# MarineRoboticsGroup/mac

Hardware: AMD Instinct MI355X
Metric: frank_wolfe_iters_per_sec (higher is better)
Workload: dtype f64; 1 GPU; configs[3]: ER N=100000 ~2M candidates, chain fixed, K=10%; N=100000, m_candidates=2001737, K=200173, fixed_edges=99999, fw_iters=209, parallelism=single GPU

## Files before the change

mac_amd/csrc/kernels.h:

```cpp
#pragma once
#include "common.h"

namespace machip {

template <typename T>
struct CsrViewT {
    int n;
    const int* rowptr;
    const int* col;
    const T* val;
};
using CsrView = CsrViewT<double>;

struct PatternView {
    int n;
    const int* prow;
    const int* pcol;
    const int* pk;
    const double* pw;
};

struct LanState {
    int jA;
    int jB;
// ... 1025 lines not shown
                                                 const double* __restrict__ cw, const double* __restrict__ v,
                                                 long lo, long hi, double* __restrict__ g, PeerVecs all = PeerVecs(),
                                                 unsigned int* __restrict__ hist0 = nullptr) {
#pragma clang fp contract(off)
    __shared__ unsigned int lh[HIST ? kBins : 1];
    if (HIST) {
        for (int i = threadIdx.x; i < kBins; i += kBlock) lh[i] = 0;
        __syncthreads();
    }
    unsigned int cur = 0xffffffffu, run = 0;
    for (long k = lo + (long)blockIdx.x * kBlock + threadIdx.x; k < hi; k += (long)gridDim.x * kBlock) {
        const double d = v[ci[k]] - v[cj[k]];
        const double t = cw[k] * d;
        const double gk = t * d;
        if (all.n) { for (int q = 0; q < all.n; ++q) peer_store(all.v[q] + k, gk); }
        else g[k] = gk;
        if (HIST) {
            const unsigned int bin = (unsigned int)(f64_key(gk) >> sel_shift(0));
            if (bin == cur) ++run;
            else { if (run) atomicAdd(&lh[cur], run); cur = bin; run = 1; }
        }
    }
    if (HIST) {
        if (run) atomicAdd(&lh[cur], run);
        __syncthreads();
        unsigned int* hr = hist0 + (size_t)(blockIdx.x % kSelRep) * kBins;
        for (int i = threadIdx.x; i < kBins; i += kBlock)
            if (lh[i]) atomicAdd(&hr[i], lh[i]);
    }
    if (all.n) peer_drain();
}

template <int BLOCK, class LoadBin>
__device__ __forceinline__ void sel_close_pass(LoadBin load_bin, int pass, unsigned long long prefix, SelState* st,
                                               unsigned int* s_w ) {
    const int tid = threadIdx.x, wv = tid >> 6, ln = tid & 63;
    const int sh = sel_shift(pass), nb = sel_bits(pass);
    const long long kk = pass ? st->kk : st->k;
    const int nbins = 1 << nb;
    constexpr int per = kBins / BLOCK;
    unsigned int c[per];
    unsigned int tsum = 0;
#pragma unroll
    for (int q = 0; q < per; ++q) {
        const int bin = nbins - 1 - (tid * per + q);
        c[q] = bin >= 0 ? load_bin(bin) : 0u;
        tsum += c[q];
    }
    unsigned int x = tsum;
    for (int o = 1; o < 64; o <<= 1) { const unsigned int y = __shfl_up(x, o, kWave); if (ln >= o) x += y; }
    __syncthreads();
    if (ln == 63) s_w[wv] = x;
    __syncthreads();
    for (int q = 0; q < wv; ++q) x += s_w[q];
    const long long pre = (long long)x;
    if (pre >= kk && pre - (long long)tsum < kk) {
        long long rem = kk - (pre - (long long)tsum);
        int q = 0;
        for (; q < per; ++q) {
            if ((long long)c[q] >= rem) break;
            rem -= c[q];
        }
        const int bin = nbins - 1 - (tid * per + q);
        st->kk = rem;
        st->prefix = (prefix << nb) | (unsigned long long)bin;
        if (pass == 5) {
            st->T = (prefix << nb) | (unsigned long long)bin;
            st->cnt_eq = (long long)c[q];
        } else if ((long long)c[q] == rem) {
            st->T = ((prefix << nb) | (unsigned long long)bin) << sh;
            st->cnt_eq = rem;
            st->ticket[7] = 1u;
        }
    }
}

__global__ __launch_bounds__(1024) void k_sel_close0(unsigned int* __restrict__ hist, SelState* st) {
    __shared__ unsigned int s_w[1024 / 64];
    if (st->k <= 0) return;
    const unsigned int* rep = hist + 6 * kBins;
    sel_close_pass<1024>([rep](int bin) {
        unsigned int v[kSelRep];
#pragma unroll
        for (int r = 0; r < kSelRep; ++r) v[r] = rep[(size_t)r * kBins + bin];
        unsigned int a = 0;
#pragma unroll
        for (int r = 0; r < kSelRep; ++r) a += v[r];
        return a; }, 0, 0ull, st, s_w);
}

template <int U, int BLOCK>
__global__ __launch_bounds__(BLOCK) void k_sel_pass(const double* __restrict__ g, long m, int pass,
                                                    unsigned int* __restrict__ hist ,
                                                    SelState* st) {
    __shared__ unsigned int lh[kBins];
    __shared__ unsigned int s_last;
    __shared__ unsigned int s_w[BLOCK / 64];
    const int tid = threadIdx.x;
    if (pass && st->ticket[7]) return;
    for (int i = tid; i < kBins; i += BLOCK) lh[i] = 0;
    __syncthreads();
    const int sh = sel_shift(pass), nb = sel_bits(pass);
// ... 37 lines not shown
__global__ __launch_bounds__(1024) void k_sel_ties(const double* __restrict__ g, long m, SelState* st, int prefer_high) {
    __shared__ int s_cnt[16];
    __shared__ long long s_found;
    const long long need = st->kk;
    const long long eq = st->cnt_eq;
    if (st->k <= 0) { if (threadIdx.x == 0) st->tie_limit = prefer_high ? 0x7fffffffffffffffll : -1; return; }
    if (need >= eq) { if (threadIdx.x == 0) st->tie_limit = prefer_high ? -1 : 0x7fffffffffffffffll; return; }
    const unsigned long long T = st->T;
    const int tid = threadIdx.x, wv = tid >> 6, ln = tid & 63;
    if (tid == 0) s_found = -1;
    long long run = 0;
    for (long base = 0; base < m; base += 1024) {
        const long ii = base + tid;
        const long i = prefer_high ? m - 1 - ii : ii;
        const bool is = ii < m && f64_key(g[i]) == T;
        const unsigned long long bal = __ballot(is);
        __syncthreads();
        if (ln == 0) s_cnt[wv] = __popcll(bal);
        __syncthreads();
        int before = 0, tot = 0;
        for (int q = 0; q < 16; ++q) { if (q < wv) before += s_cnt[q]; tot += s_cnt[q]; }
        if (run + tot >= need) {
            const int rank = before + __popcll(bal & ((1ull << ln) - 1ull));
            if (is && run + rank + 1 == need) s_found = i;
            __syncthreads();
            if (tid == 0) st->tie_limit = s_found;
            return;
        }
        run += tot;
    }
    if (tid == 0) st->tie_limit = prefer_high ? -1 : 0x7fffffffffffffffll;
}

constexpr long kSelSmallMax = 32768;
__global__ __launch_bounds__(1024) void k_sel_small(const double* __restrict__ g, long m, long long k, SelState* st, int prefer_high) {
    __shared__ unsigned int lh[kBins];
    __shared__ unsigned int s_w[16];
    __shared__ unsigned long long s_prefix, s_T;
    __shared__ long long s_kk, s_eq, s_found;
    __shared__ int s_done, s_cnt[16];
    const int tid = threadIdx.x, wv = tid >> 6, ln = tid & 63;
    if (tid == 0) { s_prefix = 0; s_T = 0; s_kk = k; s_eq = 0; s_done = 0; s_found = -1; }
    __syncthreads();
    for (int pass = 0; pass < 6 && k > 0; ++pass) {
        if (s_done) break;
        for (int i = tid; i < kBins; i += 1024) lh[i] = 0;
        __syncthreads();
        const int sh = sel_shift(pass), nb = sel_bits(pass);
        const unsigned long long prefix = s_prefix;
        const unsigned int mask = (1u << nb) - 1u;
        unsigned int cur = 0xffffffffu, run = 0;
        for (long i = tid; i < m; i += 1024) {
            const unsigned long long key = f64_key(g[i]);
            if (pass == 0 || (key >> (sh + nb)) == prefix) {
                const unsigned int bin = (unsigned int)(key >> sh) & mask;
                if (bin == cur) ++run;
                else { if (run) atomicAdd(&lh[cur], run); cur = bin; run = 1; }
            }
        }
        if (run) atomicAdd(&lh[cur], run);
        __syncthreads();
        const long long kk = s_kk;
        const int nbins = 1 << nb;
        unsigned int c[2], tsum = 0;
        for (int q = 0; q < 2; ++q) { const int bin = nbins - 1 - (tid * 2 + q); c[q] = bin >= 0 ? lh[bin] : 0u; tsum += c[q]; }
        unsigned int x = tsum;
        for (int o = 1; o < 64; o <<= 1) { const unsigned int y = __shfl_up(x, o, kWave); if (ln >= o) x += y; }
        if (ln == 63) s_w[wv] = x;
        __syncthreads();
        for (int q = 0; q < wv; ++q) x += s_w[q];
        const long long pre = (long long)x;
        if (pre >= kk && pre - (long long)tsum < kk) {
            long long rem = kk - (pre - (long long)tsum);
            int q = 0;
            for (; q < 2; ++q) { if ((long long)c[q] >= rem) break; rem -= c[q]; }
            const int bin = nbins - 1 - (tid * 2 + q);
            s_kk = rem;
            s_prefix = (prefix << nb) | (unsigned long long)bin;
            if (pass == 5) { s_T = (prefix << nb) | (unsigned long long)bin; s_eq = (long long)c[q]; }
            else if ((long long)c[q] == rem) { s_T = ((prefix << nb) | (unsigned long long)bin) << sh; s_eq = rem; s_done = 1; }
        }
        __syncthreads();
    }
    const long long need = s_kk, eq = s_eq;
    const unsigned long long T = s_T;
    if (tid == 0) {
        st->prefix = s_prefix; st->kk = need; st->cnt_eq = eq; st->T = T; st->k = k;
        for (int i = 0; i < 7; ++i) st->ticket[i] = 0;
        st->ticket[7] = (unsigned int)s_done;
    }
    if (k <= 0) { if (tid == 0) st->tie_limit = prefer_high ? 0x7fffffffffffffffll : -1; return; }
    if (need >= eq) { if (tid == 0) st->tie_limit = prefer_high ? -1 : 0x7fffffffffffffffll; return; }
    long long runs = 0;
    for (long base = 0; base < m; base += 1024) {
        const long ii = base + tid;
        const long i = prefer_high ? m - 1 - ii : ii;
        const bool is = ii < m && f64_key(g[i]) == T;
        const unsigned long long bal = __ballot(is);
        __syncthreads();
        if (ln == 0) s_cnt[wv] = __popcll(bal);
        __syncthreads();
        int before = 0, tot = 0;
        for (int q = 0; q < 16; ++q) { if (q < wv) before += s_cnt[q]; tot += s_cnt[q]; }
        if (runs + tot >= need) {
            const int rank = before + __popcll(bal & ((1ull << ln) - 1ull));
            if (is && runs + rank + 1 == need) s_found = i;
            __syncthreads();
            if (tid == 0) st->tie_limit = s_found;
            return;
        }
        runs += tot;
    }
    if (tid == 0) st->tie_limit = prefer_high ? -1 : 0x7fffffffffffffffll;
}

__global__ __launch_bounds__(kBlock) void k_fw_final(const double* __restrict__ g, const double* __restrict__ x,
                                                     long m, const SelState* __restrict__ st, double gamma,
                                                     double* __restrict__ x_next, double* __restrict__ s_out,
                                                     double* __restrict__ part ,
                                                     double tol = 0.0, unsigned long long* __restrict__ xbits_next = nullptr) {
#pragma clang fp contract(off)
    __shared__ double sm[4];
    const unsigned long long T = st->T;
    const long long lim = st->tie_limit;
    const bool none = st->k <= 0;
    double d = 0.0, q = 0.0;
    for (long i = (long)blockIdx.x * kBlock + threadIdx.x; i < m; i += (long)gridDim.x * kBlock) {
        const double gi = g[i];
        const unsigned long long key = f64_key(gi);
        const double s = (!none && (key > T || (key == T && (long long)i <= lim))) ? 1.0 : 0.0;
        if (s_out) s_out[i] = s;
        if (x) {
            const double xi = x[i];
            const double diff = s - xi;
            d += gi * diff;
            q += gi * gi;
            if (x_next) {
                const double step = gamma * diff;
                const double xn = xi + step;
                x_next[i] = xn;
                if (xbits_next) {
                    const unsigned long long bal = __ballot(xn > tol);
                    if ((threadIdx.x & 63) == 0) xbits_next[i >> 6] = bal;
                }
            }
        }
// ... 74 lines not shown
```

mac_amd/csrc/machip.hip:

```cpp
#include <rccl/rccl.h>
#include <unistd.h>

#include <algorithm>
#include <atomic>
#include <cmath>
#include <chrono>
#include <condition_variable>
#include <functional>
#include <future>
#include <memory>
#include <mutex>
#include <numeric>
#include <thread>
#include <vector>

#include "solver.h"
#include "esp.h"
#include "esp_free.h"
#include "esp_tree.h"
#include "esp_select.h"
#include "esp_relax.h"
#include "esp_exchange.h"
#include "esp_exchange_edge.h"
#include "eig_exchange.h"
// ... 51 lines not shown
    }
    void abort() {
        std::lock_guard<std::mutex> lk(mu);
        broken = true;
        cv.notify_all();
    }
};

struct machip_problem {
    int device = 0;
    hipStream_t stream = nullptr;
    int n = 0;
    long m = 0, m_pad = 0;
    double tol_sel = 1e-10;
    int *prow = nullptr, *pcol = nullptr, *pk = nullptr;
    double* pw = nullptr;
    long P = 0;
    int asm_G = 16, asm_rpb = 1, asm_grid = 1;
    int *ci = nullptr, *cj = nullptr;
    double* cw = nullptr;
    double *x = nullptr, *x_next = nullptr, *g = nullptr, *s = nullptr, *scratch_m = nullptr;
    int *cnt = nullptr, *blk_sum = nullptr, *rowptr = nullptr, *col = nullptr;
    double *val = nullptr, *blk_lnorm = nullptr;
    unsigned long long *xb = nullptr, *xb_next = nullptr;
    bool xb_valid = false, xb_next_valid = false;
    long nnz = 0, support = 0;
    int maxlen = 0;
    double lnorm = 0.0;
    bool assembled = false, have_vec = false, csr_only = false;
    bool band_dups_ok = true;
    unsigned int* hist = nullptr;
    SelState* sel = nullptr;
    double* part_fw = nullptr;
    int* h_int = nullptr;
    double* h_dbl = nullptr;
    int* d_hint = nullptr;
    double* d_hdbl = nullptr;
    Solver sol;
    ncclComm_t comm = nullptr;
    std::shared_ptr<LocalGroup> lgroup;
    bool first_collective_pending = false;
    hipEvent_t ev_g0 = nullptr, ev_g1 = nullptr, ev_g2 = nullptr;
    bool ev_g_valid = false;
    std::unique_ptr<IpcGroup> ipcg;
    int rank = 0, nranks = 1;
    bool is_lane = false, lane_fw_ready = false;
    std::vector<machip_problem*> lanes;
    unsigned long start_version = 0;
    unsigned long seen_start_version = ~0ul;

    CsrView csr() const { return CsrView{n, rowptr, col, val}; }
    PatternView pattern() const { return PatternView{n, prow, pcol, pk, pw}; }
};

static int create_lane_stream(const Options& opt, int device, hipStream_t* out) {
    if (OPT(lane_queues, 0) == 0) {
        hipDeviceProp_t prop;
        if (hipGetDeviceProperties(&prop, device) == hipSuccess && prop.multiProcessorCount > 0) {
            const int words = (prop.multiProcessorCount + 31) / 32;
            std::vector<uint32_t> mask((size_t)words, 0xffffffffu);
            if (prop.multiProcessorCount % 32) mask.back() = (1u << (prop.multiProcessorCount % 32)) - 1u;
            if (hipExtStreamCreateWithCUMask(out, (uint32_t)words, mask.data()) == hipSuccess) return MACHIP_OK;
            (void)hipGetLastError();
        }
    }
    HIP_TRY(hipStreamCreateWithFlags(out, hipStreamNonBlocking));
// ... 115 lines not shown
        p->xb_valid = true;
    }
    switch (p->asm_G) {
        case 4: launch_asm<4>(p, S); break;
        case 8: launch_asm<8>(p, S); break;
        case 16: launch_asm<16>(p, S); break;
        case 32: launch_asm<32>(p, S); break;
        default: launch_asm<64>(p, S); break;
    }
    HIP_TRY(hipGetLastError());
    const int gb = p->asm_grid;
    HIP_TRY(hipStreamSynchronize(p->stream));
    long nnz = 0, supp = 0;
    int maxlen = 0;
    double ln = 0.0;
    for (int b = 0; b < gb; ++b) {
        nnz += p->h_int[b]; supp += p->h_int[kAsmGrid + b]; maxlen = std::max(maxlen, p->h_int[2 * kAsmGrid + b]);
        ln = std::max(ln, p->h_dbl[b]);
    }
    p->nnz = nnz; p->support = supp / 2; p->lnorm = ln; p->maxlen = maxlen;
    p->assembled = true;
    return MACHIP_OK;
}

int alloc_common(machip_problem* p, int vbudget_mb = 0) {
    ST_TRY(p->sol.init(p->n, p->stream, vbudget_mb));
    HIP_TRY(hipHostMalloc((void**)&p->h_int, sizeof(int) * 3 * kAsmGrid, hipHostMallocMapped));
    HIP_TRY(hipHostMalloc((void**)&p->h_dbl, sizeof(double) * std::max(4 * kMaxGrid, kAsmGrid), hipHostMallocMapped));
    HIP_TRY(hipHostGetDevicePointer((void**)&p->d_hint, p->h_int, 0));
    HIP_TRY(hipHostGetDevicePointer((void**)&p->d_hdbl, p->h_dbl, 0));
    return MACHIP_OK;
}

int select_on(machip_problem* p, const double* keys, long k, SelState* st, int prefer_high, bool hist0_done = false) {
    const Options& opt = p->sol.opt;
    const long m = p->m;
    if (k < 0) k = 0;
    if (k > m) k = m;
    if (m <= kSelSmallMax && OPT(sel_small, 1)) {
        k_sel_small<<<1, 1024, 0, p->stream>>>(keys, m, (long long)k, st, prefer_high);
        HIP_TRY(hipGetLastError());
        return MACHIP_OK;
    }
    if (!hist0_done) k_sel_init<<<1, 1024, 0, p->stream>>>(st, (long long)k, p->hist, 6 * kBins);
    if (k > 0) {
        constexpr int B = 1024, U = 4;
        const int grid = (int)std::max<long>(1, std::min<long>(128, (m + (long)B * U - 1) / ((long)B * U)));
        if (hist0_done) k_sel_close0<<<1, 1024, 0, p->stream>>>(p->hist, st);
        for (int pass = hist0_done ? 1 : 0; pass < 6; ++pass) k_sel_pass<U, B><<<grid, B, 0, p->stream>>>(keys, m, pass, p->hist, st);
    }
    k_sel_ties<<<1, 1024, 0, p->stream>>>(keys, m, st, prefer_high);
    HIP_TRY(hipGetLastError());
    return MACHIP_OK;
}

int select_topk(machip_problem* p, long k, bool hist0_done = false) { return select_on(p, p->g, k, p->sel, 0, hist0_done); }

void shard_plan(long m, int nranks, int rank, long* lo, long* hi, long* shard) {
    const long sh = nranks > 0 ? (m + nranks - 1) / nranks : m;
    *shard = sh;
    *lo = std::min(m, sh * rank);
    *hi = std::min(m, *lo + sh);
}

int local_allgather(machip_problem* p, long shard) {
    LocalGroup& G = *p->lgroup;
    HIP_TRY(hipStreamSynchronize(p->stream));
    if (!G.barrier()) return fail(MACHIP_RCCL_ERROR, "in-process communicator was shut down by another rank");
    for (int r = 0; r < G.nranks; ++r)
        if (r != p->rank)
            HIP_TRY(hipMemcpyAsync(p->g + shard * r, G.g[(size_t)r] + shard * r, sizeof(double) * (size_t)shard,
                                   hipMemcpyDeviceToDevice, p->stream));
    HIP_TRY(hipStreamSynchronize(p->stream));
    if (!G.barrier()) return fail(MACHIP_RCCL_ERROR, "in-process communicator was shut down by another rank");
    return MACHIP_OK;
}

int compute_gradient(machip_problem* p, bool have_vec_now = false, long fuse_k = -1, bool* fused = nullptr) {
    const Options& opt = p->sol.opt;
    if (!p->have_vec && !have_vec_now) return fail(MACHIP_BAD_ARG, "no Fiedler vector on the device: call machip_fiedler first");
    const long m = p->m;
    long lo = 0, hi = m, shard = m;
    if (p->nranks > 1) shard_plan(m, p->nranks, p->rank, &lo, &hi, &shard);
    const bool ipc_gather = p->nranks > 1 && !p->comm && p->ipcg;
    if (ipc_gather) {
        k_ipc_pubwait<<<1, 64, 0, p->stream>>>(p->ipcg->view, 3);
    }
    const bool timed = p->nranks > 1;
    if (timed) {
        if (!p->ev_g0) { HIP_TRY(hipEventCreate(&p->ev_g0)); HIP_TRY(hipEventCreate(&p->ev_g1)); HIP_TRY(hipEventCreate(&p->ev_g2)); }
        p->ev_g_valid = false;
        HIP_TRY(hipEventRecord(p->ev_g0, p->stream));
    }
    if (hi > lo) {
        const int grid = (int)std::min<long>(kMaxGrid * 4, (hi - lo + kBlock - 1) / kBlock);
        PeerVecs all;
        if (ipc_gather) { all.n = p->ipcg->nranks; for (int q = 0; q < all.n; ++q) all.v[q] = p->ipcg->g[q]; }
        const bool fuse = fuse_k > 0 && p->nranks <= 1 && m > kSelSmallMax && OPT(sel_fuse, 1) != 0;
        if (fused) *fused = fuse;
        if (fuse) {
            k_sel_init<<<1, 1024, 0, p->stream>>>(p->sel, (long long)std::min(fuse_k, m), p->hist, (6 + kSelRep) * kBins);
            k_grad<true><<<grid, kBlock, 0, p->stream>>>(p->ci, p->cj, p->cw, p->sol.yvec, lo, hi, p->g, all, p->hist + 6 * kBins);
        } else k_grad<false><<<grid, kBlock, 0, p->stream>>>(p->ci, p->cj, p->cw, p->sol.yvec, lo, hi, p->g, all);
        HIP_TRY(hipGetLastError());
    }
    if (timed) HIP_TRY(hipEventRecord(p->ev_g1, p->stream));
    if (ipc_gather) {
        k_ipc_pubwait<<<1, 64, 0, p->stream>>>(p->ipcg->view, 2);
        HIP_TRY(hipGetLastError());
        HIP_TRY(hipEventRecord(p->ev_g2, p->stream));
        p->ev_g_valid = true;
        return MACHIP_OK;
    }
    if (p->nranks > 1) {
        if (p->comm) {
            NCCL_TRY(ncclAllGather(p->g + shard * p->rank, p->g, (size_t)shard, ncclDouble, p->comm, p->stream));
            if (p->first_collective_pending) {
                p->first_collective_pending = false;
                const auto t0 = std::chrono::steady_clock::now();
                const double lim = rccl_timeout_s();
                for (;;) {
                    const hipError_t q = hipStreamQuery(p->stream);
                    if (q == hipSuccess) break;
                    if (q != hipErrorNotReady) return fail(MACHIP_HIP_ERROR, std::string("first ncclAllGather: ") + hipGetErrorString(q));
                    ncclResult_t ar = ncclSuccess;
                    if (ncclCommGetAsyncError(p->comm, &ar) == ncclSuccess && ar != ncclSuccess && ar != ncclInProgress)
                        return fail(MACHIP_RCCL_ERROR, std::string("first ncclAllGather failed asynchronously: ") + ncclGetErrorString(ar));
                    if (std::chrono::duration<double>(std::chrono::steady_clock::now() - t0).count() > lim) {
                        (void)ncclCommAbort(p->comm);
                        p->comm = nullptr;
                        return fail(MACHIP_RCCL_ERROR, "first ncclAllGather of rank " + std::to_string(p->rank) + " of " + std::to_string(p->nranks) +
                                    " did not complete within " + std::to_string((int)lim) + " s: communicator aborted");
                    }
                    std::this_thread::sleep_for(std::chrono::microseconds(200));
// ... 131 lines not shown
                const int a = std::min(fi[e], fj[e]), b = std::max(fi[e], fj[e]);
                if (a >= 0 && b < n && b == a + 1 && fw[e] > 0.0) has[(size_t)a] = 1;
            }
            long cnt = 0;
            for (int64_t i = 0; i + 1 < n; ++i) cnt += has[(size_t)i];
            p->sol.chain_like = cnt >= (long)(0.98 * (double)(n - 1));
            p->sol.chain_edges = cnt;
        }
        return MACHIP_OK;
    };
    st = body();
    if (st != MACHIP_OK) { machip_destroy(p); return st; }
    *out = p;
    return MACHIP_OK;
}

void machip_destroy(machip_problem* p) {
    if (!p) return;
    for (machip_problem* q : p->lanes) machip_destroy(q);
    p->lanes.clear();
    (void)hipSetDevice(p->device);
    if (p->stream) (void)hipStreamSynchronize(p->stream);
    if (p->is_lane) { p->prow = p->pcol = p->pk = nullptr; p->pw = nullptr; p->ci = p->cj = nullptr; p->cw = nullptr; }
    if (p->comm) (void)ncclCommDestroy(p->comm);
    if (p->lgroup) p->lgroup->abort();
    if (p->ipcg) {
        IpcGroup& G = *p->ipcg;
        if (!G.clean_exit) { k_ipc_abort<<<1, 64, 0, p->stream>>>(G.view); (void)hipStreamSynchronize(p->stream); }
        p->sol.ipc = nullptr;
        p->ipcg.reset();
    }
    p->sol.destroy();
    void* ptrs[] = {p->prow, p->pcol, p->pk, p->pw, p->ci, p->cj, p->cw, p->x, p->x_next, p->g, p->s, p->scratch_m, p->cnt,
                    p->blk_sum, p->rowptr, p->col, p->val, p->blk_lnorm, p->xb, p->xb_next, p->hist, p->sel, p->part_fw};
    for (void* q : ptrs) if (q) (void)hipFree(q);
    for (hipEvent_t e : {p->ev_g0, p->ev_g1, p->ev_g2}) if (e) (void)hipEventDestroy(e);
    if (p->h_int) (void)hipHostFree(p->h_int);
    if (p->h_dbl) (void)hipHostFree(p->h_dbl);
    if (p->stream) (void)hipStreamDestroy(p->stream);
    delete p;
}

int machip_set_x(machip_problem* p, const double* x) {
    if (!p || !x || p->csr_only) return fail(MACHIP_BAD_ARG, "machip_set_x: bad handle or NULL x");
    HIP_TRY(hipSetDevice(p->device));
    HIP_TRY(hipMemcpyAsync(p->x, x, sizeof(double) * (size_t)p->m, hipMemcpyHostToDevice, p->stream));
    HIP_TRY(hipStreamSynchronize(p->stream));
    p->assembled = false; p->xb_valid = false;
    return MACHIP_OK;
}

int machip_get_x(machip_problem* p, double* x) {
    if (!p || !x || p->csr_only) return fail(MACHIP_BAD_ARG, "machip_get_x: bad handle or NULL x");
    HIP_TRY(hipSetDevice(p->device));
    HIP_TRY(hipMemcpyAsync(x, p->x, sizeof(double) * (size_t)p->m, hipMemcpyDeviceToHost, p->stream));
    HIP_TRY(hipStreamSynchronize(p->stream));
    return MACHIP_OK;
}

int machip_assemble(machip_problem* p, int64_t* nnz_out) {
    if (!p) return fail(MACHIP_BAD_ARG, "NULL handle");
    HIP_TRY(hipSetDevice(p->device));
    ST_TRY(assemble(p));
    if (nnz_out) *nnz_out = p->nnz;
    return MACHIP_OK;
}

// ... 686 lines not shown
                st = machip_fw_commit(q);
            }
            if (st == MACHIP_OK) st = machip_get_x(q, X_out + (size_t)b * m);
            if (st == MACHIP_OK && R_out) st = machip_round_nearest(q, ks[b], round_decimals, R_out + (size_t)b * m);
            upper[b] = u; iters[b] = done; status[b] = st;
            if (st != MACHIP_OK && st != MACHIP_NOT_CONVERGED && st != MACHIP_DISCONNECTED) {
                lane_status[(size_t)l] = st; lane_err[(size_t)l] = g_err;
                return;
            }
        }
    };
    std::vector<std::thread> th;
    for (int l = 1; l < nl; ++l) th.emplace_back(work, l);
    work(0);
    for (auto& t : th) t.join();
    for (int l = 0; l < nl; ++l)
        if (lane_status[(size_t)l] != MACHIP_OK) return fail((machip_status)lane_status[(size_t)l], lane_err[(size_t)l]);
    return MACHIP_OK;
}

int machip_set_option(machip_problem* p, const char* name, int64_t value) {
    const int id = option_id(name);
    if (id < 0) return fail(MACHIP_BAD_ARG, std::string("machip_set_option: unknown option '") + (name ? name : "(null)") + "'");
    const long v = value == INT64_MIN ? kOptAuto : (long)value;
    if (!p) { default_options().v[id] = v; return MACHIP_OK; }
    p->sol.opt.v[id] = v;
    for (machip_problem* q : p->lanes) q->sol.opt.v[id] = v;
    return MACHIP_OK;
}

int machip_get_option(machip_problem* p, const char* name, int64_t* value) {
    const int id = option_id(name);
    if (id < 0 || !value) return fail(MACHIP_BAD_ARG, "machip_get_option: unknown option or NULL output");
    const long v = p ? p->sol.opt.v[id] : default_options().v[id];
    *value = v == kOptAuto ? INT64_MIN : (int64_t)v;
    return MACHIP_OK;
}

const char* machip_option_name(int i) { return (i >= 0 && i < kNumOpts) ? option_names()[i] : nullptr; }

int machip_comm_timing(machip_problem* p, double* grad_us, double* exchange_us) {
    if (!p || !grad_us || !exchange_us) return fail(MACHIP_BAD_ARG, "machip_comm_timing: NULL argument");
    *grad_us = 0.0; *exchange_us = 0.0;
    if (!p->ev_g_valid) return fail(MACHIP_BAD_ARG, "machip_comm_timing: no sharded gradient has been computed on this handle");
    HIP_TRY(hipSetDevice(p->device));
    HIP_TRY(hipEventSynchronize(p->ev_g2));
    float a = 0.f, b = 0.f;
    HIP_TRY(hipEventElapsedTime(&a, p->ev_g0, p->ev_g1));
    HIP_TRY(hipEventElapsedTime(&b, p->ev_g1, p->ev_g2));
    *grad_us = 1e3 * (double)a; *exchange_us = 1e3 * (double)b;
    return MACHIP_OK;
}

int machip_solve_mode(machip_problem* p, int64_t* closures) {
    if (!p) return -1;
    if (closures) *closures = p->sol.last_wb_s;
    return p->sol.last_mode;
}

int machip_comm_drop(machip_problem* p) {
    if (!p) return fail(MACHIP_BAD_ARG, "machip_comm_drop: NULL handle");
    if (p->lgroup) return fail(MACHIP_BAD_ARG, "machip_comm_drop: in-process communicators end with their handles");
    HIP_TRY(hipSetDevice(p->device));
    (void)hipStreamSynchronize(p->stream);
    if (p->ipcg) { p->sol.ipc = nullptr; p->ipcg.reset(); }
    if (p->comm) { (void)ncclCommAbort(p->comm); p->comm = nullptr; }
// ... 343 lines not shown
```

mac_amd/csrc/options.h:

```cpp
#pragma once
#include <climits>
#include <cstdlib>
#include <cstring>
#include <mutex>
#include <string>

namespace machip {

#define MACHIP_OPTION_LIST(X)                                                                                                      \
                                                                                                          \
    X(solver) X(graph) X(debug) X(chunk) X(chunk_near) X(sched) X(near_x10) X(trigger_pct) X(classic_n) X(persist) X(pchunk)      \
    X(spec_epilogue) X(spec_slack_pct) X(f32_switch_e9) X(tailless) X(stream) X(stream_trigger_pct) X(stream_retry_pct) X(stream_look) X(stream_margin) X(stream_window) X(stream_far) X(start_land) X(start_pow) X(start_floor_e6) X(start_land_pr_permille) X(start_land_min_mean10)                                                                \
                                                                        \
    X(spmv) X(g) X(unroll) X(block) X(maxgrid) X(defer) X(tpr) X(ell)                                                              \
                                                                                                            \
    X(panel) X(panel_min_n) X(panel_min_mean10) X(panel_multi_min_mean10) X(panel_np) X(panel_nb) X(panel_b2) X(panel_g2)         \
    X(panel_cells) X(panel_maxcells) X(panel_band) X(panel_u) X(panel_u_amp) X(pan32) X(pan32_switch_e9) X(panel_ops) X(panel_rev)                                                                               \
                                                                                                 \
    X(woodbury) X(wb_max) X(wb_hard) X(wb_lane_max) X(exact_big) X(exact_switch) X(gj_look_min) X(lob_density_pct) X(lob_chunk)   \
    X(lob_patience) X(lob_small_s) X(lob_fuse)                                                                                     \
     \
    X(sel_small) X(sel_fuse) X(asm_g) X(asm_maxgrid) X(vbudget_mb) X(vcap) X(lanes) X(lane_vbudget_mb) X(lane_queues) X(shard_eig) X(ipc_panel) \
    X(rccl_timeout_s)                                                                                                              \
               \
    X(esp_free_split)                                                                                                              \
       \
    X(esp_xch_lds_kb) X(esp_xch_max_mb) X(esp_xch_profile)                                                                         \
                                                       \
    X(eig_xch_max_mb)                                                                                                              \
                                                                                                            \
    X(eig_free_rows) X(eig_free_split)

enum OptId {
#define X(n) kOpt_##n,
    MACHIP_OPTION_LIST(X)
#undef X
    kNumOpts
};

constexpr long kOptAuto = LONG_MIN;

inline const char* const* option_names() {
    static const char* const names[] = {
#define X(n) #n,
        MACHIP_OPTION_LIST(X)
#undef X
        nullptr};
    return names;
}
inline int option_id(const char* name) {
    if (!name) return -1;
    const char* const* nm = option_names();
    for (int i = 0; i < kNumOpts; ++i) if (!strcmp(nm[i], name)) return i;
    return -1;
}

// ... 43 lines not shown
```

Before: 135.1 iter/s.

## Replace multi-pass radix top-k select with two-kernel coarse bucket plus candidate list

Adds a two-kernel top-k selection path for the fused gradient histogram case. The first kernel closes pass 0 from the replicated histogram and builds a coarse 8-bit sub-histogram. The second compacts the candidates in the chosen bucket into a small global list, finishes the radix walk and tie resolution in one block, and zeroes histograms so the next iteration can skip k_sel_init. This is meant to replace several full-array radix passes and extra launches per Frank-Wolfe iteration. If the bucket holds more than the list capacity it falls back to a single-block whole-array walk, which could be slow.

Result: no change. 134.5 iter/s (-0.4%).

```diff
diff --git a/mac_amd/csrc/kernels.h b/mac_amd/csrc/kernels.h
--- a/mac_amd/csrc/kernels.h
+++ b/mac_amd/csrc/kernels.h
@@ -1081,11 +1081,9 @@
 }
 
 template <int BLOCK, class LoadBin>
-__device__ __forceinline__ void sel_close_pass(LoadBin load_bin, int pass, unsigned long long prefix, SelState* st,
-                                               unsigned int* s_w ) {
+__device__ __forceinline__ bool sel_close_find(LoadBin load_bin, int nb, long long kk, unsigned int* s_w ,
+                                               int* bin_out, long long* rem_out, unsigned int* cnt_out) {
     const int tid = threadIdx.x, wv = tid >> 6, ln = tid & 63;
-    const int sh = sel_shift(pass), nb = sel_bits(pass);
-    const long long kk = pass ? st->kk : st->k;
     const int nbins = 1 << nb;
     constexpr int per = kBins / BLOCK;
     unsigned int c[per];
@@ -1103,20 +1101,33 @@
     __syncthreads();
     for (int q = 0; q < wv; ++q) x += s_w[q];
     const long long pre = (long long)x;
-    if (pre >= kk && pre - (long long)tsum < kk) {
-        long long rem = kk - (pre - (long long)tsum);
-        int q = 0;
-        for (; q < per; ++q) {
-            if ((long long)c[q] >= rem) break;
-            rem -= c[q];
-        }
-        const int bin = nbins - 1 - (tid * per + q);
+    if (!(pre >= kk && pre - (long long)tsum < kk)) return false;
+    long long rem = kk - (pre - (long long)tsum);
+    int q = 0;
+    for (; q < per; ++q) {
+        if ((long long)c[q] >= rem) break;
+        rem -= c[q];
+    }
+    *bin_out = nbins - 1 - (tid * per + q);
+    *rem_out = rem;
+    *cnt_out = c[q];
+    return true;
+}
+
+template <int BLOCK, class LoadBin>
+__device__ __forceinline__ void sel_close_pass(LoadBin load_bin, int pass, unsigned long long prefix, SelState* st,
+                                               unsigned int* s_w ) {
+    const int sh = sel_shift(pass), nb = sel_bits(pass);
+    int bin = 0;
+    long long rem = 0;
+    unsigned int cnt = 0;
+    if (sel_close_find<BLOCK>(load_bin, nb, pass ? st->kk : st->k, s_w, &bin, &rem, &cnt)) {
         st->kk = rem;
         st->prefix = (prefix << nb) | (unsigned long long)bin;
         if (pass == 5) {
             st->T = (prefix << nb) | (unsigned long long)bin;
-            st->cnt_eq = (long long)c[q];
-        } else if ((long long)c[q] == rem) {
+            st->cnt_eq = (long long)cnt;
+        } else if ((long long)cnt == rem) {
             st->T = ((prefix << nb) | (unsigned long long)bin) << sh;
             st->cnt_eq = rem;
             st->ticket[7] = 1u;
@@ -1220,65 +1231,53 @@
     if (tid == 0) st->tie_limit = prefer_high ? -1 : 0x7fffffffffffffffll;
 }
 
-constexpr long kSelSmallMax = 32768;
-__global__ __launch_bounds__(1024) void k_sel_small(const double* __restrict__ g, long m, long long k, SelState* st, int prefer_high) {
-    __shared__ unsigned int lh[kBins];
-    __shared__ unsigned int s_w[16];
-    __shared__ unsigned long long s_prefix, s_T;
-    __shared__ long long s_kk, s_eq, s_found;
-    __shared__ int s_done, s_cnt[16];
-    const int tid = threadIdx.x, wv = tid >> 6, ln = tid & 63;
-    if (tid == 0) { s_prefix = 0; s_T = 0; s_kk = k; s_eq = 0; s_done = 0; s_found = -1; }
-    __syncthreads();
-    for (int pass = 0; pass < 6 && k > 0; ++pass) {
-        if (s_done) break;
-        for (int i = tid; i < kBins; i += 1024) lh[i] = 0;
+struct SelWalk {
+    unsigned long long prefix, T;
+    long long kk, eq, found;
+    int done;
+    unsigned int lh[kBins], s_w[16];
+    int s_cnt[16];
+};
+
+template <class KeyAt>
+__device__ __forceinline__ void sel_walk(KeyAt key_at, long cnt, int pass0, SelWalk* w) {
+    const int tid = threadIdx.x;
+    for (int pass = pass0; pass < 6; ++pass) {
+        if (w->done) break;
+        for (int i = tid; i < kBins; i += 1024) w->lh[i] = 0;
         __syncthreads();
         const int sh = sel_shift(pass), nb = sel_bits(pass);
-        const unsigned long long prefix = s_prefix;
+        const unsigned long long prefix = w->prefix;
+        const long long kk = w->kk;
         const unsigned int mask = (1u << nb) - 1u;
         unsigned int cur = 0xffffffffu, run = 0;
-        for (long i = tid; i < m; i += 1024) {
-            const unsigned long long key = f64_key(g[i]);
+        for (long i = tid; i < cnt; i += 1024) {
+            const unsigned long long key = key_at(i);
             if (pass == 0 || (key >> (sh + nb)) == prefix) {
                 const unsigned int bin = (unsigned int)(key >> sh) & mask;
                 if (bin == cur) ++run;
-                else { if (run) atomicAdd(&lh[cur], run); cur = bin; run = 1; }
+                else { if (run) atomicAdd(&w->lh[cur], run); cur = bin; run = 1; }
             }
         }
-        if (run) atomicAdd(&lh[cur], run);
+        if (run) atomicAdd(&w->lh[cur], run);
         __syncthreads();
-        const long long kk = s_kk;
-        const int nbins = 1 << nb;
-        unsigned int c[2], tsum = 0;
-        for (int q = 0; q < 2; ++q) { const int bin = nbins - 1 - (tid * 2 + q); c[q] = bin >= 0 ? lh[bin] : 0u; tsum += c[q]; }
-        unsigned int x = tsum;
-        for (int o = 1; o < 64; o <<= 1) { const unsigned int y = __shfl_up(x, o, kWave); if (ln >= o) x += y; }
-        if (ln == 63) s_w[wv] = x;
+        const unsigned int* lh = w->lh;
+        int bin = 0;
+        long long rem = 0;
+        unsigned int c = 0;
+        if (sel_close_find<1024>([lh](int b) { return lh[b]; }, nb, kk, w->s_w, &bin, &rem, &c)) {
+            w->kk = rem;
+            w->prefix = (prefix << nb) | (unsigned long long)bin;
+            if (pass == 5) { w->T = (prefix << nb) | (unsigned long long)bin; w->eq = (long long)c; }
+            else if ((long long)c == rem) { w->T = ((prefix << nb) | (unsigned long long)bin) << sh; w->eq = rem; w->done = 1; }
+        }
         __syncthreads();
-        for (int q = 0; q < wv; ++q) x += s_w[q];
-        const long long pre = (long long)x;
-        if (pre >= kk && pre - (long long)tsum < kk) {
-            long long rem = kk - (pre - (long long)tsum);
-            int q = 0;
-            for (; q < 2; ++q) { if ((long long)c[q] >= rem) break; rem -= c[q]; }
-            const int bin = nbins - 1 - (tid * 2 + q);
-            s_kk = rem;
-            s_prefix = (prefix << nb) | (unsigned long long)bin;
-            if (pass == 5) { s_T = (prefix << nb) | (unsigned long long)bin; s_eq = (long long)c[q]; }
-            else if ((long long)c[q] == rem) { s_T = ((prefix << nb) | (unsigned long long)bin) << sh; s_eq = rem; s_done = 1; }
-        }
-        __syncthreads();
-    }
-    const long long need = s_kk, eq = s_eq;
-    const unsigned long long T = s_T;
-    if (tid == 0) {
-        st->prefix = s_prefix; st->kk = need; st->cnt_eq = eq; st->T = T; st->k = k;
-        for (int i = 0; i < 7; ++i) st->ticket[i] = 0;
-        st->ticket[7] = (unsigned int)s_done;
-    }
-    if (k <= 0) { if (tid == 0) st->tie_limit = prefer_high ? 0x7fffffffffffffffll : -1; return; }
-    if (need >= eq) { if (tid == 0) st->tie_limit = prefer_high ? -1 : 0x7fffffffffffffffll; return; }
+    }
+}
+
+__device__ __forceinline__ void sel_ties_scan(const double* __restrict__ g, long m, unsigned long long T, long long need,
+                                              int prefer_high, SelWalk* w, SelState* st) {
+    const int tid = threadIdx.x, wv = tid >> 6, ln = tid & 63;
     long long runs = 0;
     for (long base = 0; base < m; base += 1024) {
         const long ii = base + tid;
@@ -1286,20 +1285,224 @@
         const bool is = ii < m && f64_key(g[i]) == T;
         const unsigned long long bal = __ballot(is);
         __syncthreads();
-        if (ln == 0) s_cnt[wv] = __popcll(bal);
+        if (ln == 0) w->s_cnt[wv] = __popcll(bal);
         __syncthreads();
         int before = 0, tot = 0;
-        for (int q = 0; q < 16; ++q) { if (q < wv) before += s_cnt[q]; tot += s_cnt[q]; }
+        for (int q = 0; q < 16; ++q) { if (q < wv) before += w->s_cnt[q]; tot += w->s_cnt[q]; }
         if (runs + tot >= need) {
             const int rank = before + __popcll(bal & ((1ull << ln) - 1ull));
-            if (is && runs + rank + 1 == need) s_found = i;
+            if (is && runs + rank + 1 == need) w->found = i;
             __syncthreads();
-            if (tid == 0) st->tie_limit = s_found;
+            if (tid == 0) st->tie_limit = w->found;
             return;
         }
         runs += tot;
     }
     if (tid == 0) st->tie_limit = prefer_high ? -1 : 0x7fffffffffffffffll;
+}
+
+__device__ __forceinline__ void sel_whole(const double* __restrict__ g, long m, long long k, int pass0, int prefer_high,
+                                          SelWalk* w, SelState* st) {
+    const int tid = threadIdx.x;
+    if (k > 0) sel_walk([g](long i) { return f64_key(g[i]); }, m, pass0, w);
+    const long long need = w->kk, eq = w->eq;
+    const unsigned long long T = w->T;
+    if (tid == 0) {
+        st->prefix = w->prefix; st->kk = need; st->cnt_eq = eq; st->T = T; st->k = k;
+        for (int i = 0; i < 7; ++i) st->ticket[i] = 0;
+        st->ticket[7] = (unsigned int)w->done;
+    }
+    if (k <= 0) { if (tid == 0) st->tie_limit = prefer_high ? 0x7fffffffffffffffll : -1; return; }
+    if (need >= eq) { if (tid == 0) st->tie_limit = prefer_high ? -1 : 0x7fffffffffffffffll; return; }
+    sel_ties_scan(g, m, T, need, prefer_high, w, st);
+}
+
+constexpr long kSelSmallMax = 32768;
+__global__ __launch_bounds__(1024) void k_sel_small(const double* __restrict__ g, long m, long long k, SelState* st, int prefer_high) {
+    __shared__ SelWalk w;
+    if (threadIdx.x == 0) { w.prefix = 0; w.T = 0; w.kk = k; w.eq = 0; w.done = 0; w.found = -1; }
+    __syncthreads();
+    sel_whole(g, m, k, 0, prefer_high, &w, st);
+}
+
+constexpr int kSelList = 8192;
+constexpr int kSelCoarse = 8;
+struct SelTwo {
+    unsigned int cursor;
+    unsigned int ticket_a, ticket_b;
+    unsigned int whole;
+    unsigned int whole_runs;
+    unsigned int bucket;
+    unsigned int cprefix;
+    long long ckk;
+};
+
+template <int U, int BLOCK>
+__global__ __launch_bounds__(BLOCK) void k_sel_two_a(const double* __restrict__ g, long m, long long k,
+                                                      unsigned int* __restrict__ hist , SelState* st, SelTwo* tw) {
+    constexpr int kCoarse = 1 << kSelCoarse;
+    __shared__ unsigned int lh[kCoarse];
+    __shared__ unsigned int s_w[BLOCK / 64];
+    __shared__ unsigned int s_last, s_cnt[2];
+    __shared__ int s_bin[2];
+    __shared__ long long s_rem[2];
+    const int tid = threadIdx.x;
+    const unsigned int* rep = hist + 6 * kBins;
+    unsigned int* gh = hist + kBins;
+    {
+        int bin = 0;
+        long long rem = 0;
+        unsigned int cnt = 0;
+        if (sel_close_find<BLOCK>([rep](int b) {
+                unsigned int v[kSelRep];
+#pragma unroll
+                for (int r = 0; r < kSelRep; ++r) v[r] = rep[(size_t)r * kBins + b];
+                unsigned int a = 0;
+#pragma unroll
+                for (int r = 0; r < kSelRep; ++r) a += v[r];
+                return a; }, sel_bits(0), k, s_w, &bin, &rem, &cnt)) { s_bin[0] = bin; s_rem[0] = rem; s_cnt[0] = cnt; }
+    }
+    for (int i = tid; i < kCoarse; i += BLOCK) lh[i] = 0;
+    __syncthreads();
+    const unsigned long long bin0 = (unsigned long long)s_bin[0];
+    const long long rem0 = s_rem[0];
+    const bool done0 = (long long)s_cnt[0] == rem0;
+    if (!done0) {
+        constexpr int sh = 53 - kSelCoarse;
+        unsigned int cur = 0xffffffffu, run = 0;
+        for (long i0 = (long)blockIdx.x * (BLOCK * U) + tid; i0 < m; i0 += (long)gridDim.x * (BLOCK * U)) {
+            double gv[U];
+#pragma unroll
+            for (int q = 0; q < U; ++q) { const long i = i0 + (long)q * BLOCK; gv[q] = g[i < m ? i : m - 1]; }
+#pragma unroll
+            for (int q = 0; q < U; ++q) {
+                if (i0 + (long)q * BLOCK >= m) continue;
+                const unsigned long long key = f64_key(gv[q]);
+                if ((key >> 53) == bin0) {
+                    const unsigned int bin = (unsigned int)(key >> sh) & (kCoarse - 1);
+                    if (bin == cur) ++run;
+                    else { if (run) atomicAdd(&lh[cur], run); cur = bin; run = 1; }
+                }
+            }
+        }
+        if (run) atomicAdd(&lh[cur], run);
+        __syncthreads();
+        unsigned int seen = 0;
+        for (int i = tid; i < kCoarse; i += BLOCK)
+            if (lh[i]) seen |= __hip_atomic_fetch_add(&gh[i], lh[i], __ATOMIC_RELAXED, __HIP_MEMORY_SCOPE_AGENT);
+        asm volatile("" ::"v"(seen));
+    }
+    __syncthreads();
+    if (tid == 0)
+        s_last = (__hip_atomic_fetch_add(&tw->ticket_a, 1u, __ATOMIC_ACQ_REL, __HIP_MEMORY_SCOPE_AGENT) == gridDim.x - 1);
+    __syncthreads();
+    if (!s_last) return;
+    if (!done0) {
+        int bin = 0;
+        long long rem = 0;
+        unsigned int cnt = 0;
+        if (sel_close_find<BLOCK>([gh](int b) { return __hip_atomic_load(&gh[b], __ATOMIC_RELAXED, __HIP_MEMORY_SCOPE_AGENT); },
+                                  kSelCoarse, rem0, s_w, &bin, &rem, &cnt)) { s_bin[1] = bin; s_rem[1] = rem; s_cnt[1] = cnt; }
+    }
+    __syncthreads();
+    for (int i = tid; i < kCoarse; i += BLOCK) gh[i] = 0u;
+    if (tid == 0) {
+        st->prefix = bin0; st->kk = rem0; st->k = k;
+        st->cnt_eq = done0 ? rem0 : 0; st->T = done0 ? bin0 << 53 : 0ull;
+        st->tie_limit = done0 ? 0x7fffffffffffffffll : -1;
+        for (int i = 0; i < 7; ++i) st->ticket[i] = 0;
+        st->ticket[7] = done0 ? 1u : 0u;
+        const unsigned int bucket = done0 ? 0u : s_cnt[1];
+        const unsigned int whole = bucket > (unsigned int)kSelList ? 1u : 0u;
+        tw->whole = whole;
+        tw->whole_runs += whole;
+        tw->bucket = bucket;
+        tw->cprefix = done0 ? 0u : (unsigned int)((bin0 << kSelCoarse) | (unsigned long long)s_bin[1]);
+        tw->ckk = done0 ? 0 : s_rem[1];
+        tw->ticket_a = 0u;
+    }
+}
+
+template <int U, int BLOCK>
+__global__ __launch_bounds__(BLOCK) void k_sel_two_b(const double* __restrict__ g, long m, unsigned int* __restrict__ hist, SelState* st,
+                                                      SelTwo* tw, unsigned long long* lkey , unsigned int* lidx ) {
+    static_assert(BLOCK == 1024, "sel_walk is written for 1 024 threads");
+    __shared__ SelWalk w;
+    __shared__ unsigned int s_idx[kSelList];
+    __shared__ unsigned int s_last, s_n, s_base;
+    const int tid = threadIdx.x, ln = tid & 63;
+    for (int i = blockIdx.x * BLOCK + tid; i < kSelRep * kBins; i += gridDim.x * BLOCK) hist[6 * kBins + i] = 0u;
+    if (st->ticket[7]) return;
+    if (tid == 0) { w.prefix = st->prefix; w.T = 0; w.kk = st->kk; w.eq = 0; w.done = 0; w.found = -1; s_n = 0; }
+    if (tw->whole) {
+        if (blockIdx.x) return;
+        __syncthreads();
+        sel_whole(g, m, st->k, 1, 0, &w, st);
+        return;
+    }
+    __syncthreads();
+    const unsigned long long cprefix = tw->cprefix;
+    for (long i0 = (long)blockIdx.x * (BLOCK * U) + tid; i0 < m; i0 += (long)gridDim.x * (BLOCK * U)) {
+        double gv[U];
+#pragma unroll
+        for (int q = 0; q < U; ++q) { const long i = i0 + (long)q * BLOCK; gv[q] = g[i < m ? i : m - 1]; }
+#pragma unroll
+        for (int q = 0; q < U; ++q) {
+            const long i = i0 + (long)q * BLOCK;
+            const bool hit = i < m && (f64_key(gv[q]) >> (53 - kSelCoarse)) == cprefix;
+            const unsigned long long bal = __ballot(hit);
+            if (bal == 0ull) continue;
+            const int lead = __ffsll((long long)bal) - 1;
+            unsigned int base = 0;
+            if (ln == lead) base = atomicAdd(&s_n, (unsigned int)__popcll(bal));
+            base = __shfl(base, lead, kWave);
+            const unsigned int slot = base + (unsigned int)__popcll(bal & ((1ull << ln) - 1ull));
+            if (hit && slot < (unsigned int)kSelList) s_idx[slot] = (unsigned int)i;
+        }
+    }
+    __syncthreads();
+    const unsigned int mine = s_n < (unsigned int)kSelList ? s_n : (unsigned int)kSelList;
+    if (tid == 0 && mine) s_base = __hip_atomic_fetch_add(&tw->cursor, mine, __ATOMIC_RELAXED, __HIP_MEMORY_SCOPE_AGENT);
+    __syncthreads();
+    unsigned int seen = 0;
+    for (unsigned int a = tid; a < mine; a += BLOCK) {
+        const unsigned int slot = s_base + a, i = s_idx[a];
+        if (slot < (unsigned int)kSelList) {
+            seen |= (unsigned int)__hip_atomic_exchange(&lkey[slot], f64_key(g[i]), __ATOMIC_RELAXED, __HIP_MEMORY_SCOPE_AGENT);
+            seen |= __hip_atomic_exchange(&lidx[slot], i, __ATOMIC_RELAXED, __HIP_MEMORY_SCOPE_AGENT);
+        }
+    }
+    asm volatile("" ::"v"(seen));
+    __syncthreads();
+    if (tid == 0)
+        s_last = (__hip_atomic_fetch_add(&tw->ticket_b, 1u, __ATOMIC_ACQ_REL, __HIP_MEMORY_SCOPE_AGENT) == gridDim.x - 1);
+    __syncthreads();
+    if (!s_last) return;
+    const unsigned int filled = __hip_atomic_load(&tw->cursor, __ATOMIC_RELAXED, __HIP_MEMORY_SCOPE_AGENT);
+    const long cnt = (long)(filled < (unsigned int)kSelList ? filled : (unsigned int)kSelList);
+    if (tid == 0) { w.kk = tw->ckk; s_n = 0; }
+    __syncthreads();
+    sel_walk([lkey](long i) { return __hip_atomic_load(&lkey[i], __ATOMIC_RELAXED, __HIP_MEMORY_SCOPE_AGENT); }, cnt, 1, &w);
+    const long long need = w.kk, eq = w.eq;
+    const unsigned long long T = w.T;
+    if (tid == 0) {
+        st->prefix = w.prefix; st->kk = need; st->cnt_eq = eq; st->T = T;
+        st->ticket[7] = (unsigned int)w.done;
+        tw->cursor = 0u; tw->ticket_b = 0u;
+        if (need >= eq) st->tie_limit = 0x7fffffffffffffffll;
+    }
+    if (need >= eq) return;
+    for (long i = tid; i < cnt; i += BLOCK)
+        if (__hip_atomic_load(&lkey[i], __ATOMIC_RELAXED, __HIP_MEMORY_SCOPE_AGENT) == T)
+            s_idx[atomicAdd(&s_n, 1u)] = __hip_atomic_load(&lidx[i], __ATOMIC_RELAXED, __HIP_MEMORY_SCOPE_AGENT);
+    __syncthreads();
+    const unsigned int nt = s_n;
+    for (unsigned int a = tid; a < nt; a += BLOCK) {
+        const unsigned int me = s_idx[a];
+        long long below = 0;
+        for (unsigned int b = 0; b < nt; ++b) below += s_idx[b] < me;
+        if (below + 1 == need) st->tie_limit = (long long)me;
+    }
 }
 
 __global__ __launch_bounds__(kBlock) void k_fw_final(const double* __restrict__ g, const double* __restrict__ x,
diff --git a/mac_amd/csrc/machip.hip b/mac_amd/csrc/machip.hip
--- a/mac_amd/csrc/machip.hip
+++ b/mac_amd/csrc/machip.hip
@@ -107,6 +107,12 @@
     unsigned int* hist = nullptr;
     SelState* sel = nullptr;
     double* part_fw = nullptr;
+    SelTwo* sel2 = nullptr;
+    unsigned long long* sel_lkey = nullptr;
+    unsigned int* sel_lidx = nullptr;
+    bool sel_clean = false;
+    bool sel_two_armed = false;
+    long sel_two_runs = 0;
     int* h_int = nullptr;
     double* h_dbl = nullptr;
     int* d_hint = nullptr;
@@ -288,6 +294,16 @@
     return MACHIP_OK;
 }
 
+int alloc_select(machip_problem* p) {
+    if (!p->sel_lkey) ST_TRY(dev_alloc(&p->sel_lkey, kSelList));
+    if (!p->sel_lidx) ST_TRY(dev_alloc(&p->sel_lidx, kSelList));
+    if (!p->sel2) {
+        ST_TRY(dev_alloc(&p->sel2, 1));
+        HIP_TRY(hipMemsetAsync(p->sel2, 0, sizeof(SelTwo), p->stream));
+    }
+    return MACHIP_OK;
+}
+
 int select_on(machip_problem* p, const double* keys, long k, SelState* st, int prefer_high, bool hist0_done = false) {
     const Options& opt = p->sol.opt;
     const long m = p->m;
@@ -298,6 +314,19 @@
         HIP_TRY(hipGetLastError());
         return MACHIP_OK;
     }
+    const bool two = hist0_done && p->sel_two_armed && k > 0 && prefer_high == 0 && st == p->sel;
+    p->sel_two_armed = false;
+    if (two) {
+        constexpr int B = 1024, U = 4;
+        const int grid = (int)std::max<long>(1, std::min<long>(128, (m + (long)B * U - 1) / ((long)B * U)));
+        k_sel_two_a<U, B><<<grid, B, 0, p->stream>>>(keys, m, (long long)k, p->hist, st, p->sel2);
+        k_sel_two_b<U, B><<<grid, B, 0, p->stream>>>(keys, m, p->hist, st, p->sel2, p->sel_lkey, p->sel_lidx);
+        HIP_TRY(hipGetLastError());
+        ++p->sel_two_runs;
+        p->sel_clean = true;
+        return MACHIP_OK;
+    }
+    p->sel_clean = false;
     if (!hist0_done) k_sel_init<<<1, 1024, 0, p->stream>>>(st, (long long)k, p->hist, 6 * kBins);
     if (k > 0) {
         constexpr int B = 1024, U = 4;
@@ -355,7 +384,12 @@
         const bool fuse = fuse_k > 0 && p->nranks <= 1 && m > kSelSmallMax && OPT(sel_fuse, 1) != 0;
         if (fused) *fused = fuse;
         if (fuse) {
-            k_sel_init<<<1, 1024, 0, p->stream>>>(p->sel, (long long)std::min(fuse_k, m), p->hist, (6 + kSelRep) * kBins);
+            const bool two = OPT(sel_two, 1) != 0;
+            if (two && !p->sel2) ST_TRY(alloc_select(p));
+            if (!two || !p->sel_clean)
+                k_sel_init<<<1, 1024, 0, p->stream>>>(p->sel, (long long)std::min(fuse_k, m), p->hist, (6 + kSelRep) * kBins);
+            p->sel_clean = false;
+            p->sel_two_armed = two;
             k_grad<true><<<grid, kBlock, 0, p->stream>>>(p->ci, p->cj, p->cw, p->sol.yvec, lo, hi, p->g, all, p->hist + 6 * kBins);
         } else k_grad<false><<<grid, kBlock, 0, p->stream>>>(p->ci, p->cj, p->cw, p->sol.yvec, lo, hi, p->g, all);
         HIP_TRY(hipGetLastError());
@@ -553,7 +587,8 @@
     }
     p->sol.destroy();
     void* ptrs[] = {p->prow, p->pcol, p->pk, p->pw, p->ci, p->cj, p->cw, p->x, p->x_next, p->g, p->s, p->scratch_m, p->cnt,
-                    p->blk_sum, p->rowptr, p->col, p->val, p->blk_lnorm, p->xb, p->xb_next, p->hist, p->sel, p->part_fw};
+                    p->blk_sum, p->rowptr, p->col, p->val, p->blk_lnorm, p->xb, p->xb_next, p->hist, p->sel, p->part_fw,
+                    p->sel2, p->sel_lkey, p->sel_lidx};
     for (void* q : ptrs) if (q) (void)hipFree(q);
     for (hipEvent_t e : {p->ev_g0, p->ev_g1, p->ev_g2}) if (e) (void)hipEventDestroy(e);
     if (p->h_int) (void)hipHostFree(p->h_int);
@@ -1306,6 +1341,17 @@
 int machip_get_option(machip_problem* p, const char* name, int64_t* value) {
     const int id = option_id(name);
     if (id < 0 || !value) return fail(MACHIP_BAD_ARG, "machip_get_option: unknown option or NULL output");
+    if (p && (id == kOpt_sel_two_runs || id == kOpt_sel_whole_runs)) {
+        SelTwo h;
+        memset(&h, 0, sizeof(h));
+        if (id == kOpt_sel_whole_runs && p->sel2) {
+            HIP_TRY(hipSetDevice(p->device));
+            HIP_TRY(hipMemcpyAsync(&h, p->sel2, sizeof(SelTwo), hipMemcpyDeviceToHost, p->stream));
+            HIP_TRY(hipStreamSynchronize(p->stream));
+        }
+        *value = id == kOpt_sel_two_runs ? (int64_t)p->sel_two_runs : (int64_t)h.whole_runs;
+        return MACHIP_OK;
+    }
     const long v = p ? p->sol.opt.v[id] : default_options().v[id];
     *value = v == kOptAuto ? INT64_MIN : (int64_t)v;
     return MACHIP_OK;
diff --git a/mac_amd/csrc/options.h b/mac_amd/csrc/options.h
--- a/mac_amd/csrc/options.h
+++ b/mac_amd/csrc/options.h
@@ -20,8 +20,9 @@
     X(woodbury) X(wb_max) X(wb_hard) X(wb_lane_max) X(exact_big) X(exact_switch) X(gj_look_min) X(lob_density_pct) X(lob_chunk)   \
     X(lob_patience) X(lob_small_s) X(lob_fuse)                                                                                     \
      \
-    X(sel_small) X(sel_fuse) X(asm_g) X(asm_maxgrid) X(vbudget_mb) X(vcap) X(lanes) X(lane_vbudget_mb) X(lane_queues) X(shard_eig) X(ipc_panel) \
+    X(sel_small) X(sel_fuse) X(sel_two) X(sel_two_runs) X(sel_whole_runs) X(asm_g) X(asm_maxgrid) X(vbudget_mb) X(vcap) X(lanes) X(lane_vbudget_mb) X(lane_queues) X(shard_eig) X(ipc_panel) \
     X(rccl_timeout_s)                                                                                                              \
+     \
                \
     X(esp_free_split)                                                                                                              \
        \
```
